# PaddlePaddle/PaddleNLP

Measured on AMD Instinct MI355X. Metric: tokens_per_sec_whole_node_llama3_8b_pretrain, higher is better.
Workload: dtype bf16; 1 GPU; model=llama3-8b, global_batch=8, seq_len=4096, parallelism=single, recompute=False

## Files before the change

### paddlenlp_amd/ops/csrc/bindings.cpp

```cpp
#include <torch/extension.h>
#include <ATen/hip/HIPContext.h>
#include <vector>

#include "launchers.h"

#define CHECK_GPU(x) TORCH_CHECK(x.is_cuda(), #x " must be on GPU")
#define CHECK_CONTIG(x) TORCH_CHECK(x.is_contiguous(), #x " must be contiguous")
#define CHECK_BF16(x) TORCH_CHECK(x.scalar_type() == torch::kBFloat16, #x " must be bf16")

static hipStream_t cur_stream() {
    return at::hip::getCurrentHIPStream().stream();
}

std::vector<torch::Tensor> rms_norm_fwd(torch::Tensor x, torch::Tensor w, double eps) {
    CHECK_GPU(x); CHECK_CONTIG(x); CHECK_BF16(x); CHECK_BF16(w);
    int H = x.size(-1);
    TORCH_CHECK(H % 8 == 0, "hidden size must be a multiple of 8");
    long long rows = x.numel() / H;
    auto y = torch::empty_like(x);
    auto invrms = torch::empty({rows}, x.options().dtype(torch::kFloat32));
    launch_rms_norm_fwd(x.data_ptr(), w.data_ptr(), y.data_ptr(),
                        invrms.data_ptr<float>(), rows, H, (float)eps, cur_stream());
    return {y, invrms};
}
// ... 141 lines not shown
        pre_lens.data_ptr<int>(), seq_lens.data_ptr<int>(),
        reinterpret_cast<const long long*>(eos_ids.data_ptr<int64_t>()),
        (int)eos_ids.numel(), not_need_stop.data_ptr<int>(),
        max_new ? max_new->data_ptr<int>() : nullptr,
        (long long)pad_id, B, (int)pre_ids.size(1), cur_stream());
}

void block_step(torch::Tensor block_table, torch::Tensor seq_lens,
                torch::Tensor stop_flags, torch::Tensor active,
                torch::Tensor free_list, torch::Tensor free_count,
                torch::Tensor is_block_step, int64_t block_size) {
    int B = block_table.size(0);
    launch_block_step(block_table.data_ptr<int>(), seq_lens.data_ptr<int>(),
                      stop_flags.data_ptr<signed char>(), active.data_ptr<signed char>(),
                      free_list.data_ptr<int>(), free_count.data_ptr<int>(),
                      is_block_step.data_ptr<signed char>(), B, (int)block_size,
                      (int)block_table.size(1), cur_stream());
}

torch::Tensor mfma32_probe(torch::Tensor A, torch::Tensor B) {
    CHECK_GPU(A); CHECK_BF16(A);
    auto C = torch::empty({32, 32}, A.options().dtype(torch::kFloat32));
    launch_mfma32_probe(A.contiguous().data_ptr(), B.contiguous().data_ptr(),
                        C.data_ptr<float>(), cur_stream());
    return C;
}

std::vector<torch::Tensor> permlane_probe() {
    auto opt = torch::TensorOptions().dtype(torch::kInt32).device(torch::kCUDA);
    auto o0 = torch::empty({64}, opt);
    auto o1 = torch::empty({64}, opt);
    launch_permlane_probe(o0.data_ptr<int>(), o1.data_ptr<int>(), cur_stream());
    return {o0, o1};
}

static void check_attn_args(const torch::Tensor& q, const torch::Tensor& k,
                            const torch::Tensor& v,
                            const torch::Tensor* dout = nullptr,
                            const torch::Tensor* o = nullptr,
                            const torch::Tensor* lse = nullptr,
                            const torch::Tensor* startend = nullptr) {
    auto check4d = [](const torch::Tensor& t, const char* name) {
        TORCH_CHECK(t.is_cuda(), name, " must be on GPU");
        TORCH_CHECK(t.scalar_type() == torch::kBFloat16, name, " must be bf16");
        TORCH_CHECK(t.is_contiguous(), name, " must be contiguous");
        TORCH_CHECK(t.dim() == 4, name, " must be [B,S,H,D]");
    };
    check4d(q, "q");
    check4d(k, "k");
    check4d(v, "v");
    int64_t B = q.size(0), Sq = q.size(1), Hq = q.size(2), D = q.size(3);
    int64_t Skv = k.size(1), Hk = k.size(2);
    TORCH_CHECK(D == 128 || D == 64 || D == 32, "head dim must be 32/64/128, got ", D);
    TORCH_CHECK(k.sizes() == v.sizes(), "k and v shapes must agree");
    TORCH_CHECK(k.size(0) == B && k.size(3) == D, "k/v must be [B,Skv,Hk,D] matching q");
    TORCH_CHECK(Hk > 0 && Hq % Hk == 0, "GQA requires Hq % Hk == 0");
    if (dout) {
        check4d(*dout, "dout");
        TORCH_CHECK(dout->sizes() == q.sizes(), "dout must be shaped like q");
    }
    if (o) {
        check4d(*o, "o");
        TORCH_CHECK(o->sizes() == q.sizes(), "o must be shaped like q");
    }
    if (lse) {
        TORCH_CHECK(lse->is_cuda() && lse->is_contiguous() &&
// ... 22 lines not shown
}

std::vector<torch::Tensor> flash_attn_fwd(torch::Tensor q, torch::Tensor k, torch::Tensor v,
                                          bool causal) {
    return flash_attn_fwd_ex(q, k, v, causal, false);
}

std::vector<torch::Tensor> flash_attn_bwd_ex(torch::Tensor dout, torch::Tensor q,
                                             torch::Tensor k, torch::Tensor v,
                                             torch::Tensor o, torch::Tensor lse,
                                             bool causal, bool force_v1) {
    check_attn_args(q, k, v, &dout, &o, &lse);
    int B = q.size(0), Sq = q.size(1), Hq = q.size(2), D = q.size(3);
    int Skv = k.size(1), Hk = k.size(2);
    auto dq = torch::empty_like(q);
    auto dk_h = torch::empty({B, Skv, Hk, D}, k.options());
    auto dv_h = torch::empty({B, Skv, Hk, D}, v.options());
    auto delta = torch::empty({B, Hq, Sq}, q.options().dtype(torch::kFloat32));
    float scale = 1.0f / std::sqrt((float)D);
    launch_flash_bwd(dout.data_ptr(), q.data_ptr(), k.data_ptr(), v.data_ptr(),
                     o.data_ptr(), lse.data_ptr<float>(), delta.data_ptr<float>(),
                     dq.data_ptr(), dk_h.data_ptr(), dv_h.data_ptr(),
                     B, Sq, Skv, Hq, Hk, D, scale, causal, force_v1, cur_stream());
    return {dq, dk_h, dv_h};
}

std::vector<torch::Tensor> flash_attn_bwd(torch::Tensor dout, torch::Tensor q,
                                          torch::Tensor k, torch::Tensor v,
                                          torch::Tensor o, torch::Tensor lse,
                                          bool causal) {
    return flash_attn_bwd_ex(dout, q, k, v, o, lse, causal, false);
}

void fused_adamw(std::vector<torch::Tensor> params, std::vector<torch::Tensor> grads,
                 std::vector<torch::Tensor> exp_avgs, std::vector<torch::Tensor> exp_avg_sqs,
                 std::vector<torch::Tensor> masters,
                 double lr, double beta1, double beta2, double eps, double wd,
                 int64_t step) {
    TORCH_CHECK(!params.empty());
    bool has_master = !masters.empty();
    const long long CHUNK = 1 << 22;
    std::vector<AdamWChunk> chunks;
    for (size_t i = 0; i < params.size(); i++) {
        auto& p = params[i];
        CHECK_GPU(p); CHECK_CONTIG(p);
        bool is_bf16 = p.scalar_type() == torch::kBFloat16;
        TORCH_CHECK(!is_bf16 || has_master, "bf16 params need master weights");
        long long n = p.numel();
        torch::Tensor g = grads[i];
        if (g.scalar_type() != p.scalar_type()) g = g.to(p.scalar_type());
        for (long long off = 0; off < n; off += CHUNK) {
            AdamWChunk c;
            c.param = p.data_ptr();
            c.grad = g.data_ptr();
            c.m = exp_avgs[i].data_ptr<float>();
            c.v = exp_avg_sqs[i].data_ptr<float>();
            c.master = has_master ? masters[i].data_ptr<float>() : nullptr;
            c.offset = off;
            c.n = std::min(CHUNK, n - off);
            c.is_bf16 = is_bf16 ? 1 : 0;
            chunks.push_back(c);
        }
    }
    auto meta = torch::from_blob(chunks.data(), {(long long)(chunks.size() * sizeof(AdamWChunk))},
                                 torch::kUInt8).clone();
    auto dev_meta = meta.to(params[0].device(), true);
// ... 136 lines not shown
    TORCH_CHECK(K % 8 == 0, "K must be a multiple of 8");
    auto y = torch::empty({R, (long)K}, x.options().dtype(torch::kFloat8_e4m3fn));
    auto scales = torch::empty({R}, x.options().dtype(torch::kFloat32));
    launch_fp8_rowwise_quant(x2.data_ptr(), y.data_ptr(), scales.data_ptr<float>(),
                             R, K, cur_stream());
    return {y, scales};
}

torch::Tensor wint8_gemv(torch::Tensor x, torch::Tensor wq, torch::Tensor scale) {
    CHECK_GPU(x); CHECK_BF16(x);
    auto x2 = x.contiguous().view({-1, x.size(-1)});
    int M = x2.size(0), K = x2.size(1), N = wq.size(0);
    TORCH_CHECK(M <= 16, "wint8_gemv is for decode shapes (M <= 16)");
    TORCH_CHECK(K % 128 == 0, "K must be a multiple of 128");
    auto sizes = x.sizes().vec();
    sizes.back() = N;
    auto y = torch::empty(sizes, x.options());
    launch_wint8_gemv(x2.data_ptr(), wq.data_ptr(), scale.data_ptr<float>(),
                      y.data_ptr(), M, N, K, cur_stream());
    return y;
}

PYBIND11_MODULE(TORCH_EXTENSION_NAME, m) {
    m.def("rms_norm_fwd", &rms_norm_fwd);
    m.def("rms_norm_bwd", &rms_norm_bwd);
    m.def("rope_fwd", &rope_fwd);
    m.def("swiglu_fwd", &swiglu_fwd);
    m.def("swiglu_bwd", &swiglu_bwd);
    m.def("cross_entropy_fwd", &cross_entropy_fwd);
    m.def("cross_entropy_bwd", &cross_entropy_bwd);
    m.def("mfma_probe", &mfma_probe);
    m.def("mfma32_probe", &mfma32_probe);
    m.def("permlane_probe", &permlane_probe);
    m.def("apply_repetition_penalty", &apply_repetition_penalty);
    m.def("topp_sample", &topp_sample,
          py::arg("logits"), py::arg("temperature"), py::arg("top_p"),
          py::arg("uniform"), py::arg("ban_eos") = py::none(),
          py::arg("cur_lens") = py::none(), py::arg("min_lens") = py::none());
    m.def("decode_update", &decode_update,
          py::arg("tokens"), py::arg("stop_flags"), py::arg("active"),
          py::arg("pre_ids"), py::arg("pre_lens"), py::arg("seq_lens"),
          py::arg("eos_ids"), py::arg("not_need_stop"),
          py::arg("max_new") = py::none(), py::arg("pad_id") = 0);
    m.def("block_step", &block_step);
    m.def("flash_attn_fwd", &flash_attn_fwd);
    m.def("flash_attn_fwd_ex", &flash_attn_fwd_ex);
    m.def("flash_attn_bwd", &flash_attn_bwd);
    m.def("flash_attn_bwd_ex", &flash_attn_bwd_ex);
    m.def("flashmask_attn_fwd", &flashmask_attn_fwd);
    m.def("flashmask_attn_bwd", &flashmask_attn_bwd);
    m.def("fused_adamw", &fused_adamw);
    m.def("paged_decode_attn", &paged_decode_attn,
          py::arg("q"), py::arg("k_cache"), py::arg("v_cache"),
          py::arg("block_table"), py::arg("seq_lens"),
          py::arg("k_scale") = c10::nullopt, py::arg("v_scale") = c10::nullopt);
    m.def("rope_cache_append", &rope_cache_append,
          py::arg("qkv"), py::arg("k_cache"), py::arg("v_cache"),
          py::arg("block_table"), py::arg("seq_lens_before"),
          py::arg("cos_t"), py::arg("sin_t"), py::arg("Hq"), py::arg("Hk"),
          py::arg("token_counts") = c10::nullopt,
          py::arg("k_scale") = c10::nullopt, py::arg("v_scale") = c10::nullopt);
    m.def("wint8_gemv", &wint8_gemv);
    m.def("fp8_rowwise_quant", &fp8_rowwise_quant);
    m.def("skinny_gemm", &skinny_gemm, py::arg("x"), py::arg("w"),
          py::arg("ksplit") = 8);
}
// ... 1 lines not shown
```

### paddlenlp_amd/ops/csrc/flash_attn_bwd_v2.hip

```cpp
#include "launchers.h"
#include "mfma.h"

#define FB2_WAVES 8
#define FB2_BLOCK (FB2_WAVES * 64)

template <int D, bool MASKED = false>
__global__ __launch_bounds__(FB2_BLOCK) void flash_bwd2_dq_kernel(
    const ushort_t* __restrict__ q, const ushort_t* __restrict__ k,
    const ushort_t* __restrict__ v, const ushort_t* __restrict__ dout,
    const float* __restrict__ lse, const float* __restrict__ delta,
    ushort_t* __restrict__ dq, const int* __restrict__ startend,
    int B, int Sq, int Skv, int Hq, int Hk, float scale, int causal) {
    constexpr int BLKN = 64;
    constexpr int DSTEPS = D / 16;
    constexpr int NDT = D / 32;
    constexpr int BLKM = FB2_WAVES * 32;

    __shared__ ushort_t k_lds[2][BLKN * D];
    __shared__ ushort_t v_lds[2][BLKN * D];
    __shared__ ushort_t kt_lds[2][D * BLKN];
    __shared__ int se_lds[2][MASKED ? BLKN : 1];

    const int tid = threadIdx.x;
    const int wave = tid >> 6;
    const int lane = tid & 63;
    const int l32 = lane & 31;
    const int hi = lane >> 5;

    int qt, bh;
    if ((gridDim.y & 7) == 0) {
        const int flat = blockIdx.x + gridDim.x * blockIdx.y;
        const int idx = flat >> 3;
        qt = idx % gridDim.x;
        bh = (flat & 7) * (gridDim.y >> 3) + idx / gridDim.x;
    } else {
        qt = blockIdx.x;
        bh = blockIdx.y;
    }
    const int b = bh / Hq, hq = bh % Hq;
    const int hk = hq / (Hq / Hk);
    const int q_base = qt * BLKM;
    const int qw = q_base + wave * 32;
    const int qg = qw + l32;
    const int causal_off = Skv - Sq;

    const long long q_row_stride = (long long)Hq * D;
    const long long kv_row_stride = (long long)Hk * D;
    const ushort_t* q_ptr = q + ((long long)b * Sq * Hq + hq) * D;
    const ushort_t* do_ptr = dout + ((long long)b * Sq * Hq + hq) * D;
    const ushort_t* k_ptr = k + ((long long)b * Skv * Hk + hk) * D;
    const ushort_t* v_ptr = v + ((long long)b * Skv * Hk + hk) * D;

    frag8 aq[DSTEPS], ado[DSTEPS];
    float lse_q = INFINITY, dl_q = 0.f;
    if (qg < Sq) {
#pragma unroll
        for (int kk = 0; kk < DSTEPS; kk++) {
            aq[kk] = *reinterpret_cast<const frag8*>(
                q_ptr + (long long)qg * q_row_stride + kk * 16 + hi * 8);
            ado[kk] = *reinterpret_cast<const frag8*>(
                do_ptr + (long long)qg * q_row_stride + kk * 16 + hi * 8);
        }
        lse_q = lse[((long long)b * Hq + hq) * Sq + qg];
        dl_q = delta[((long long)b * Hq + hq) * Sq + qg];
    } else {
#pragma unroll
        for (int kk = 0; kk < DSTEPS; kk++) { aq[kk] = frag8{0}; ado[kk] = frag8{0}; }
    }

    f32x16 acc_dq[NDT];
#pragma unroll
// ... 113 lines not shown
            if (MASKED) {
                se_max_next = tile_se_max(kv_base + BLKN);
                stage_skip = (q_base >= se_max_next);
            }
            if (!stage_skip) load_tile(kv_base + BLKN);
        }
        if (!wave_skip) process_sub(1);

        if (kvt + 1 < n_kv_tiles && !stage_skip)
            write_tile(cur ^ 1, kv_base + BLKN);
        if (MASKED) se_max_cur = se_max_next;
        __syncthreads();
    }

#pragma unroll
    for (int r = 0; r < 16; r++) {
        int qrow = qw + crow32(r, hi);
        if (qrow >= Sq) continue;
        ushort_t* dqr = dq + ((long long)b * Sq + qrow) * q_row_stride + (long long)hq * D;
#pragma unroll
        for (int n = 0; n < NDT; n++)
            dqr[n * 32 + l32] = f32_to_bf16(acc_dq[n][r]);
    }
}

template <int D, bool MASKED = false>
__global__ __launch_bounds__(FB2_BLOCK, 1) void flash_bwd2_dkv_kernel(
    const ushort_t* __restrict__ q, const ushort_t* __restrict__ k,
    const ushort_t* __restrict__ v, const ushort_t* __restrict__ dout,
    const float* __restrict__ lse, const float* __restrict__ delta,
    ushort_t* __restrict__ dk, ushort_t* __restrict__ dv,
    const int* __restrict__ startend,
    int B, int Sq, int Skv, int Hq, int Hk, float scale, int causal) {
    constexpr int BLKQ = 64;
    constexpr int DSTEPS = D / 16;
    constexpr int NDT = D / 32;
    constexpr int BLKKV = FB2_WAVES * 32;

    __shared__ ushort_t q_lds[2][BLKQ * D];
    __shared__ ushort_t do_lds[2][BLKQ * D];
    __shared__ ushort_t qt_lds[2][D * BLKQ];
    __shared__ ushort_t dot_lds[2][D * BLKQ];
    __shared__ float lse_lds[2][BLKQ];
    __shared__ float dl_lds[2][BLKQ];

    const int tid = threadIdx.x;
    const int wave = tid >> 6;
    const int lane = tid & 63;
    const int l32 = lane & 31;
    const int hi = lane >> 5;

    int kvt, bh;
    if ((gridDim.y & 7) == 0) {
        const int flat = blockIdx.x + gridDim.x * blockIdx.y;
        const int idx = flat >> 3;
        kvt = idx % gridDim.x;
        bh = (flat & 7) * (gridDim.y >> 3) + idx / gridDim.x;
    } else {
        kvt = blockIdx.x;
        bh = blockIdx.y;
    }
    const int b = bh / Hk, hk = bh % Hk;
    const int G = Hq / Hk;
    const int kv_base = kvt * BLKKV;
    const int kvw = kv_base + wave * 32;
    const int kvg_lane = kvw + l32;
    const int causal_off = Skv - Sq;
    __shared__ int blk_max_lds[MASKED ? FB2_WAVES : 1];
    int kv_end_lane = 0x7fffffff;
    int wave_max_end = 0x7fffffff;
    int block_max_end = 0x7fffffff;
    if (MASKED) {
        kv_end_lane = (kvg_lane < Skv)
            ? startend[(long long)b * Skv + kvg_lane] : 0;
        wave_max_end = kv_end_lane;
#pragma unroll
        for (int off = 32; off; off >>= 1)
            wave_max_end = max(wave_max_end,
                               __shfl_xor(wave_max_end, off, 64));
        if (lane == 0) blk_max_lds[wave] = wave_max_end;
    }

    const long long q_row_stride = (long long)Hq * D;
    const long long kv_row_stride = (long long)Hk * D;
    const ushort_t* k_ptr = k + ((long long)b * Skv * Hk + hk) * D;
    const ushort_t* v_ptr = v + ((long long)b * Skv * Hk + hk) * D;

    frag8 bk[DSTEPS], bv[DSTEPS];
    if (kvg_lane < Skv) {
#pragma unroll
        for (int kk = 0; kk < DSTEPS; kk++) {
            bk[kk] = *reinterpret_cast<const frag8*>(
                k_ptr + (long long)kvg_lane * kv_row_stride + kk * 16 + hi * 8);
            bv[kk] = *reinterpret_cast<const frag8*>(
                v_ptr + (long long)kvg_lane * kv_row_stride + kk * 16 + hi * 8);
        }
    } else {
#pragma unroll
        for (int kk = 0; kk < DSTEPS; kk++) { bk[kk] = frag8{0}; bv[kk] = frag8{0}; }
    }

    f32x16 acc_dk[NDT], acc_dv[NDT];
#pragma unroll
    for (int n = 0; n < NDT; n++)
#pragma unroll
        for (int r = 0; r < 16; r++) { acc_dk[n][r] = 0.f; acc_dv[n][r] = 0.f; }

    int qt0 = 0;
    if (causal) qt0 = max(0, (kv_base - causal_off) / BLKQ);
    const int n_q_tiles = (Sq + BLKQ - 1) / BLKQ;

    const int s_rowp = tid >> 4;
    const int s_col = (tid & 15) * 8;
    const int s_row0 = s_rowp * 2;
    short8v sq0, sq1, sd0, sd1;

    for (int g = 0; g < G; g++) {
        const int hq = hk * G + g;
        const ushort_t* q_ptr = q + ((long long)b * Sq * Hq + hq) * D;
        const ushort_t* do_ptr = dout + ((long long)b * Sq * Hq + hq) * D;
        const float* lse_row = lse + ((long long)b * Hq + hq) * Sq;
        const float* dl_row = delta + ((long long)b * Hq + hq) * Sq;

        auto load_qtile = [&](int q_tb) {
            int g0 = q_tb + s_row0;
            sq0 = short8v{0,0,0,0,0,0,0,0}; sq1 = sq0; sd0 = sq0; sd1 = sq0;
            if (g0 < Sq) {
                sq0 = *reinterpret_cast<const short8v*>(q_ptr + (long long)g0 * q_row_stride + s_col);
                sd0 = *reinterpret_cast<const short8v*>(do_ptr + (long long)g0 * q_row_stride + s_col);
            }
            if (g0 + 1 < Sq) {
                sq1 = *reinterpret_cast<const short8v*>(q_ptr + (long long)(g0 + 1) * q_row_stride + s_col);
                sd1 = *reinterpret_cast<const short8v*>(do_ptr + (long long)(g0 + 1) * q_row_stride + s_col);
            }
        };
        auto write_qtile = [&](int q_tb, int buf) {
            *reinterpret_cast<short8v*>(swz<D>(q_lds[buf], s_row0, s_col)) = sq0;
            *reinterpret_cast<short8v*>(swz<D>(q_lds[buf], s_row0 + 1, s_col)) = sq1;
            *reinterpret_cast<short8v*>(swz<D>(do_lds[buf], s_row0, s_col)) = sd0;
            *reinterpret_cast<short8v*>(swz<D>(do_lds[buf], s_row0 + 1, s_col)) = sd1;
#pragma unroll
            for (int j = 0; j < 8; j++) {
                unsigned pq = ((unsigned)(unsigned short)sq0[j]) |
                              (((unsigned)(unsigned short)sq1[j]) << 16);
                unsigned pd = ((unsigned)(unsigned short)sd0[j]) |
                              (((unsigned)(unsigned short)sd1[j]) << 16);
                *reinterpret_cast<unsigned*>(swz<BLKQ>(qt_lds[buf], s_col + j, s_row0)) = pq;
                *reinterpret_cast<unsigned*>(swz<BLKQ>(dot_lds[buf], s_col + j, s_row0)) = pd;
            }
            if (tid < BLKQ) {
                int qgl = q_tb + tid;
                lse_lds[buf][tid] = (qgl < Sq) ? lse_row[qgl] : INFINITY;
                dl_lds[buf][tid] = (qgl < Sq) ? dl_row[qgl] : 0.f;
            }
        };

        load_qtile(qt0 * BLKQ);
        write_qtile(qt0 * BLKQ, qt0 & 1);
        __syncthreads();
        if (MASKED) {
            block_max_end = blk_max_lds[0];
#pragma unroll
            for (int w = 1; w < FB2_WAVES; w++)
                block_max_end = max(block_max_end, blk_max_lds[w]);
        }

        for (int qt = qt0; qt < n_q_tiles; qt++) {
            const int q_tb = qt * BLKQ;
            const int cur = qt & 1;
            bool wave_skip =
                causal && (q_tb + BLKQ - 1 + causal_off < kvw);
            if (MASKED && q_tb >= wave_max_end) wave_skip = true;

            if (!wave_skip) {
#pragma unroll 1
                for (int sub = 0; sub < 2; sub++) {
                    f32x16 st, dp;
#pragma unroll
                    for (int r = 0; r < 16; r++) { st[r] = 0.f; dp[r] = 0.f; }
                    __builtin_amdgcn_s_setprio(1);
#pragma unroll
                    for (int kk = 0; kk < DSTEPS; kk++) {
                        frag8 aqf = *reinterpret_cast<const frag8*>(
                            swz<D>(q_lds[cur], sub * 32 + l32, kk * 16 + hi * 8));
                        frag8 adf = *reinterpret_cast<const frag8*>(
                            swz<D>(do_lds[cur], sub * 32 + l32, kk * 16 + hi * 8));
                        st = mfma32(aqf, bk[kk], st);
                        dp = mfma32(adf, bv[kk], dp);
                    }
                    __builtin_amdgcn_s_setprio(0);

#pragma unroll
                    for (int r = 0; r < 16; r++) {
                        int qrow = sub * 32 + crow32(r, hi);
                        int qgl = q_tb + qrow;
                        float ls = lse_lds[cur][qrow];
                        float dl = dl_lds[cur][qrow];
                        bool vis = (qgl < Sq) && (kvg_lane < Skv) &&
                                   (!causal || kvg_lane <= qgl + causal_off);
                        if (MASKED) vis = vis && (qgl < kv_end_lane);
                        float p = (vis && ls != INFINITY)
                                      ? __expf(st[r] * scale - ls) : 0.f;
                        st[r] = p;
                        dp[r] = p * (dp[r] - dl) * scale;
                    }

                    __builtin_amdgcn_s_setprio(1);
#pragma unroll
                    for (int ksl = 0; ksl < 2; ksl++) {
                        const int ks = sub * 2 + ksl;
                        frag8 apt = t12_convert(st, ksl * 8);
                        frag8 ads = t12_convert(dp, ksl * 8);
#pragma unroll
                        for (int n = 0; n < NDT; n++) {
                            frag8 bdo = *reinterpret_cast<const frag8*>(
                                swz<BLKQ>(dot_lds[cur], n * 32 + l32, ks * 16 + hi * 8));
                            frag8 bq = *reinterpret_cast<const frag8*>(
                                swz<BLKQ>(qt_lds[cur], n * 32 + l32, ks * 16 + hi * 8));
                            acc_dv[n] = mfma32(apt, bdo, acc_dv[n]);
                            acc_dk[n] = mfma32(ads, bq, acc_dk[n]);
                        }
                    }
                    __builtin_amdgcn_s_setprio(0);
                }
            }

            if (qt + 1 < n_q_tiles &&
                !(MASKED && q_tb + BLKQ >= block_max_end)) {
                load_qtile(q_tb + BLKQ);
                write_qtile(q_tb + BLKQ, cur ^ 1);
            }
            __syncthreads();
        }
        __syncthreads();
    }

    const long long out_row_stride = (long long)Hk * D;
#pragma unroll
    for (int r = 0; r < 16; r++) {
        int kvr = kvw + crow32(r, hi);
        if (kvr >= Skv) continue;
        long long base = ((long long)b * Skv + kvr) * out_row_stride + (long long)hk * D;
#pragma unroll
        for (int n = 0; n < NDT; n++) {
            dk[base + n * 32 + l32] = f32_to_bf16(acc_dk[n][r]);
            dv[base + n * 32 + l32] = f32_to_bf16(acc_dv[n][r]);
        }
    }
}

bool launch_flash_bwd2(const void* dout, const void* q, const void* k, const void* v,
                       const void* o, const float* lse, float* delta,
                       void* dq, void* dk, void* dv,
                       int B, int Sq, int Skv, int Hq, int Hk, int D,
                       float scale, bool causal, hipStream_t stream) {
    if (D != 128 || (Hq % Hk) != 0) return false;
    launch_flash_bwd_delta(dout, o, delta, B, Sq, Hq, D, stream);
    dim3 gq((Sq + 255) / 256, B * Hq);
    hipLaunchKernelGGL((flash_bwd2_dq_kernel<128, false>), gq, dim3(FB2_BLOCK), 0, stream,
                       (const ushort_t*)q, (const ushort_t*)k, (const ushort_t*)v,
                       (const ushort_t*)dout, lse, delta, (ushort_t*)dq,
                       (const int*)nullptr,
                       B, Sq, Skv, Hq, Hk, scale, causal ? 1 : 0);
    dim3 gkv((Skv + 255) / 256, B * Hk);
    hipLaunchKernelGGL((flash_bwd2_dkv_kernel<128, false>), gkv, dim3(FB2_BLOCK), 0, stream,
                       (const ushort_t*)q, (const ushort_t*)k, (const ushort_t*)v,
                       (const ushort_t*)dout, lse, delta, (ushort_t*)dk, (ushort_t*)dv,
                       (const int*)nullptr,
                       B, Sq, Skv, Hq, Hk, scale, causal ? 1 : 0);
    return true;
}

bool launch_flash_bwd2_mask(const void* dout, const void* q, const void* k,
                            const void* v, const void* o, const float* lse,
                            float* delta, void* dq, void* dk, void* dv,
                            const int* startend,
                            int B, int Sq, int Skv, int Hq, int Hk, int D,
                            float scale, hipStream_t stream) {
    if (D != 128 || (Hq % Hk) != 0) return false;
    launch_flash_bwd_delta(dout, o, delta, B, Sq, Hq, D, stream);
    dim3 gq((Sq + 255) / 256, B * Hq);
    hipLaunchKernelGGL((flash_bwd2_dq_kernel<128, true>), gq, dim3(FB2_BLOCK), 0, stream,
                       (const ushort_t*)q, (const ushort_t*)k, (const ushort_t*)v,
                       (const ushort_t*)dout, lse, delta, (ushort_t*)dq, startend,
                       B, Sq, Skv, Hq, Hk, scale, 1);
    dim3 gkv((Skv + 255) / 256, B * Hk);
    hipLaunchKernelGGL((flash_bwd2_dkv_kernel<128, true>), gkv, dim3(FB2_BLOCK), 0, stream,
                       (const ushort_t*)q, (const ushort_t*)k, (const ushort_t*)v,
                       (const ushort_t*)dout, lse, delta, (ushort_t*)dk, (ushort_t*)dv,
                       startend, B, Sq, Skv, Hq, Hk, scale, 1);
    return true;
}
```

### paddlenlp_amd/ops/csrc/flash_attn_v2.hip

```cpp
#include "launchers.h"
#include "mfma.h"

#define FA2_WAVES 8
#define FA2_BLOCK (FA2_WAVES * 64)
#define FA2_BLKN 64
#define FA2_QW 32
#define FA2_BLKM (FA2_WAVES * FA2_QW)
#define DEFER_THR 8.0f

__global__ void mfma32_layout_probe(const ushort_t* A, const ushort_t* B, float* C) {
    int l = threadIdx.x;
    int l32 = l & 31, hi = l >> 5;
    frag8 a, b;
#pragma unroll
    for (int j = 0; j < 8; j++) {
        a[j] = (short)A[l32 * 16 + hi * 8 + j];
        b[j] = (short)B[(hi * 8 + j) * 32 + l32];
    }
    f32x16 c;
#pragma unroll
    for (int r = 0; r < 16; r++) c[r] = 0.f;
    c = mfma32(a, b, c);
#pragma unroll
    for (int r = 0; r < 16; r++) C[crow32(r, hi) * 32 + l32] = c[r];
// ... 1 lines not shown

__global__ void permlane_probe(int* out0, int* out1) {
    int l = threadIdx.x;
    auto r = __builtin_amdgcn_permlane32_swap((unsigned)l, (unsigned)(1000 + l),
                                              false, false);
    out0[l] = (int)r[0];
    out1[l] = (int)r[1];
}

template <int D, bool MASKED = false>
__global__ __launch_bounds__(FA2_BLOCK) void flash_fwd2_kernel(
    const ushort_t* __restrict__ q,
    const ushort_t* __restrict__ k,
    const ushort_t* __restrict__ v,
    ushort_t* __restrict__ o,
    float* __restrict__ lse,
    const int* __restrict__ startend,
    int B, int Sq, int Skv, int Hq, int Hk, float scale, int causal) {
    constexpr int DSTEPS = D / 16;
    constexpr int NDT = D / 32;
    constexpr int KVT = FA2_BLKN / 32;

    __shared__ ushort_t k_lds[2][FA2_BLKN * D];
    __shared__ ushort_t vt_lds[2][D * FA2_BLKN];
    __shared__ int se_lds[2][MASKED ? FA2_BLKN : 1];

    const int tid = threadIdx.x;
    const int wave = tid >> 6;
    const int lane = tid & 63;
    const int l32 = lane & 31;
    const int hi = lane >> 5;

    int qt, bh;
    if ((gridDim.y & 7) == 0) {
        const int flat = blockIdx.x + gridDim.x * blockIdx.y;
        const int idx = flat >> 3;
        qt = idx % gridDim.x;
        bh = (flat & 7) * (gridDim.y >> 3) + idx / gridDim.x;
    } else {
        qt = blockIdx.x;
        bh = blockIdx.y;
    }
    const int b = bh / Hq, hq = bh % Hq;
    const int hk = hq / (Hq / Hk);
    const int q_base = qt * FA2_BLKM;
    const int qw = q_base + wave * FA2_QW;
    const int qg = qw + l32;
    const int causal_off = Skv - Sq;

    const long long q_row_stride = (long long)Hq * D;
    const long long kv_row_stride = (long long)Hk * D;
    const ushort_t* q_ptr = q + ((long long)b * Sq * Hq + hq) * D;
    const ushort_t* k_ptr = k + ((long long)b * Skv * Hk + hk) * D;
    const ushort_t* v_ptr = v + ((long long)b * Skv * Hk + hk) * D;

    frag8 aq[DSTEPS];
    if (qg < Sq) {
#pragma unroll
        for (int kk = 0; kk < DSTEPS; kk++)
            aq[kk] = *reinterpret_cast<const frag8*>(
                q_ptr + (long long)qg * q_row_stride + kk * 16 + hi * 8);
    } else {
#pragma unroll
        for (int kk = 0; kk < DSTEPS; kk++) aq[kk] = frag8{0};
    }

    float m_run = -INFINITY, l_run = 0.f;
    f32x16 acc_o[NDT];
#pragma unroll
    for (int n = 0; n < NDT; n++)
#pragma unroll
        for (int r = 0; r < 16; r++) acc_o[n][r] = 0.f;

    int n_kv_tiles = (Skv + FA2_BLKN - 1) / FA2_BLKN;
    if (causal) {
// ... 236 lines not shown
```

### paddlenlp_amd/ops/csrc/launchers.h

```cpp
#pragma once

#include <hip/hip_runtime_api.h>

#include <stdexcept>
#include <string>

[[noreturn]] inline void unsupported_head_dim(const char* op, int D) {
    throw std::runtime_error(std::string(op) + ": no kernel for head dim " +
                             std::to_string(D));
}

void launch_rms_norm_fwd(const void* x, const void* w, void* y, float* invrms,
                         long long rows, int H, float eps, hipStream_t stream);
void launch_rms_norm_bwd(const void* dy, const void* x, const void* w,
                         const float* invrms, void* dx, float* dw_partial,
                         float* dw32, void* dw, bool dw_is_bf16,
                         long long rows, int H, int P, hipStream_t stream);
void launch_rope(const void* x, void* out, const float* cos_t, const float* sin_t,
                 long long n_rows, int H, int D, int S, bool backward,
                 hipStream_t stream);
void launch_swiglu_fwd(const void* x, void* y, long long N, int I, hipStream_t stream);
void launch_swiglu_bwd(const void* dy, const void* x, void* dx, long long N, int I,
                       hipStream_t stream);
void launch_ce_fwd(const void* logits, const long long* labels, float* loss,
// ... 10 lines not shown
    float* v;
    float* master;
    long long offset;
    long long n;
    int is_bf16;
};
void launch_adamw(const AdamWChunk* dev_chunks, int n_chunks,
                  float lr, float beta1, float beta2, float eps, float wd,
                  float bias1, float bias2, hipStream_t stream);

void launch_mfma_probe(const void* A, const void* B, float* C, hipStream_t stream);
void launch_flash_fwd(const void* q, const void* k, const void* v, void* o,
                      float* lse, int B, int Sq, int Skv, int Hq, int Hk, int D,
                      float scale, bool causal, bool force_v1, hipStream_t stream);
void launch_flash_bwd(const void* dout, const void* q, const void* k, const void* v,
                      const void* o, const float* lse, float* delta,
                      void* dq, void* dk, void* dv,
                      int B, int Sq, int Skv, int Hq, int Hk, int D,
                      float scale, bool causal, bool force_v1, hipStream_t stream);
void launch_flash_fwd_mask(const void* q, const void* k, const void* v, void* o,
                           float* lse, const int* startend,
                           int B, int Sq, int Skv, int Hq, int Hk, int D,
                           float scale, hipStream_t stream);
void launch_flash_bwd_mask(const void* dout, const void* q, const void* k, const void* v,
                           const void* o, const float* lse, float* delta,
                           void* dq, void* dk, void* dv, const int* startend,
                           int B, int Sq, int Skv, int Hq, int Hk, int D,
                           float scale, hipStream_t stream);
void launch_flash_bwd_delta(const void* dout, const void* o, float* delta,
                            int B, int Sq, int Hq, int D, hipStream_t stream);

void launch_mfma32_probe(const void* A, const void* B, float* C, hipStream_t stream);
void launch_permlane_probe(int* out0, int* out1, hipStream_t stream);
bool launch_flash_fwd2(const void* q, const void* k, const void* v, void* o,
                       float* lse, int B, int Sq, int Skv, int Hq, int Hk,
                       int D, float scale, bool causal, hipStream_t stream);
bool launch_flash_fwd2_mask(const void* q, const void* k, const void* v,
                            void* o, float* lse, const int* startend,
                            int B, int Sq, int Skv, int Hq, int Hk,
                            int D, float scale, hipStream_t stream);
bool launch_flash_bwd2(const void* dout, const void* q, const void* k, const void* v,
                       const void* o, const float* lse, float* delta,
                       void* dq, void* dk, void* dv,
                       int B, int Sq, int Skv, int Hq, int Hk, int D,
                       float scale, bool causal, hipStream_t stream);
bool launch_flash_bwd2_mask(const void* dout, const void* q, const void* k,
                            const void* v, const void* o, const float* lse,
                            float* delta, void* dq, void* dk, void* dv,
                            const int* startend,
                            int B, int Sq, int Skv, int Hq, int Hk, int D,
                            float scale, hipStream_t stream);

int paged_decode_nsplit(int B, int Hk);
void launch_paged_decode_attn(const void* q, const void* k_cache, const void* v_cache,
                              const float* k_scale, const float* v_scale,
                              const int* block_table, const int* seq_lens, void* out,
                              float* partials, int nsplit,
                              int B, int Hq, int Hk, int D, int block_size,
                              int max_blocks, float scale, int cache_mode,
                              hipStream_t stream);
bool launch_paged_decode_attn3(const void* q, const void* k_cache, const void* v_cache,
                               const float* k_scale, const float* v_scale,
                               const int* block_table, const int* seq_lens, void* out,
                               float* partials, int nsplit,
                               int B, int Hq, int Hk, int D, int block_size,
                               int max_blocks, float scale, int cache_mode,
                               hipStream_t stream);
void launch_rope_cache_append(const void* qkv, void* q_out, void* k_cache, void* v_cache,
                              float* k_scale, float* v_scale,
                              const int* block_table, const int* seq_lens_before,
                              const float* cos_t, const float* sin_t,
                              int B, int T, int Hq, int Hk, int D, int block_size,
                              int max_blocks, const int* token_counts,
                              int cache_mode, hipStream_t stream);

void launch_wint8_gemv(const void* x, const void* wq, const float* scale, void* y,
                       int M, int N, int K, hipStream_t stream);
void launch_fp8_rowwise_quant(const void* x, void* y, float* scales,
// ... 24 lines not shown
```

### paddlenlp_amd/ops/csrc/mfma.h

```cpp
#pragma once

#include "common.h"

typedef short8v frag8;

__device__ __forceinline__ f32x4 mfma16(frag8 a, frag8 b, f32x4 c) {
    return __builtin_amdgcn_mfma_f32_16x16x32_bf16(a, b, c, 0, 0, 0);
}

__device__ __forceinline__ f32x16 mfma32(frag8 a, frag8 b, f32x16 c) {
    return __builtin_amdgcn_mfma_f32_32x32x16_bf16(a, b, c, 0, 0, 0);
}

__device__ __forceinline__ int crow32(int r, int hi) {
    return (r & 3) + 8 * (r >> 2) + 4 * hi;
}

template <int LD>
__device__ __forceinline__ char* swz(ushort_t* base, int row, int col_elem) {
    return reinterpret_cast<char*>(base) +
           (((row * LD + col_elem) * 2) ^ ((row & 7) << 4));
}

__device__ __forceinline__ unsigned pack_bf16(float a, float b) {
    return (unsigned)f32_to_bf16(a) | ((unsigned)f32_to_bf16(b) << 16);
}

__device__ __forceinline__ frag8 t12_convert(const f32x16& p, int rb) {
    unsigned w[4];
    {
        unsigned lo0 = pack_bf16(p[rb + 0], p[rb + 1]);
        unsigned hi0 = pack_bf16(p[rb + 4], p[rb + 5]);
        auto rr = __builtin_amdgcn_permlane32_swap(lo0, hi0, false, false);
        w[0] = rr[0]; w[2] = rr[1];
    }
    {
        unsigned lo1 = pack_bf16(p[rb + 2], p[rb + 3]);
        unsigned hi1 = pack_bf16(p[rb + 6], p[rb + 7]);
        auto rr = __builtin_amdgcn_permlane32_swap(lo1, hi1, false, false);
        w[1] = rr[0]; w[3] = rr[1];
    }
    frag8 f;
#pragma unroll
    for (int j = 0; j < 4; j++) {
        f[j * 2] = (short)(w[j] & 0xffff);
        f[j * 2 + 1] = (short)(w[j] >> 16);
    }
    return f;
}
```

Measured before the change: 19380 tokens/s.

## Use LDS DMA and transpose reads in flash bwd dKV; regroup XCD tile order

The dK/dV backward kernel now fills one swizzled shared-memory image per Q and dO tile using direct global-to-LDS DMA loads. It reads transposed fragments with ds_read_tr16 instead of storing separate row and transposed copies through registers. The loop over heads and Q tiles is flattened into one double-buffered pipeline that prefetches the next tile, and the masked case computes the upper bound on Q tiles once. Block-to-tile mapping across XCDs is regrouped so head groups are interleaved, with descending tile order for forward and dQ and ascending for dKV. A probe kernel and a parts-selectable backward entry point are also added.

Measured after the change: 21080 tokens/s (median of 6 runs). +8.7%, better.

```diff
diff --git a/paddlenlp_amd/ops/csrc/bindings.cpp b/paddlenlp_amd/ops/csrc/bindings.cpp
--- a/paddlenlp_amd/ops/csrc/bindings.cpp
+++ b/paddlenlp_amd/ops/csrc/bindings.cpp
@@ -197,6 +197,18 @@
     auto o1 = torch::empty({64}, opt);
     launch_permlane_probe(o0.data_ptr<int>(), o1.data_ptr<int>(), cur_stream());
     return {o0, o1};
+}
+
+std::vector<torch::Tensor> lds_image_probe(torch::Tensor X) {
+    CHECK_GPU(X); CHECK_BF16(X);
+    TORCH_CHECK(X.dim() == 2 && X.size(0) == 64 && X.size(1) == 128,
+                "lds_image_probe: X must be [64,128]");
+    auto Xc = X.contiguous();
+    auto out_row = torch::empty_like(Xc);
+    auto out_tr = torch::empty_like(Xc);
+    launch_lds_image_probe(Xc.data_ptr(), out_row.data_ptr(), out_tr.data_ptr(),
+                           cur_stream());
+    return {out_row, out_tr};
 }
 
 static void check_attn_args(const torch::Tensor& q, const torch::Tensor& k,
@@ -285,6 +297,31 @@
     return flash_attn_bwd_ex(dout, q, k, v, o, lse, causal, false);
 }
 
+std::vector<torch::Tensor> flash_attn_bwd2_parts(torch::Tensor dout, torch::Tensor q,
+                                                 torch::Tensor k, torch::Tensor v,
+                                                 torch::Tensor o, torch::Tensor lse,
+                                                 torch::Tensor delta, bool causal,
+                                                 int64_t parts) {
+    check_attn_args(q, k, v, &dout, &o, &lse);
+    TORCH_CHECK(delta.is_cuda() && delta.is_contiguous() &&
+                    delta.scalar_type() == torch::kFloat32 &&
+                    delta.sizes() == lse.sizes(),
+                "delta must be a contiguous fp32 GPU tensor shaped like lse");
+    int B = q.size(0), Sq = q.size(1), Hq = q.size(2), D = q.size(3);
+    int Skv = k.size(1), Hk = k.size(2);
+    auto dq = torch::empty_like(q);
+    auto dk_h = torch::empty({B, Skv, Hk, D}, k.options());
+    auto dv_h = torch::empty({B, Skv, Hk, D}, v.options());
+    float scale = 1.0f / std::sqrt((float)D);
+    TORCH_CHECK(launch_flash_bwd2(dout.data_ptr(), q.data_ptr(), k.data_ptr(),
+                                  v.data_ptr(), o.data_ptr(), lse.data_ptr<float>(),
+                                  delta.data_ptr<float>(), dq.data_ptr(),
+                                  dk_h.data_ptr(), dv_h.data_ptr(), B, Sq, Skv, Hq,
+                                  Hk, D, scale, causal, cur_stream(), (int)parts),
+                "flash_attn_bwd2_parts: no v2 kernel for this shape");
+    return {dq, dk_h, dv_h};
+}
+
 void fused_adamw(std::vector<torch::Tensor> params, std::vector<torch::Tensor> grads,
                  std::vector<torch::Tensor> exp_avgs, std::vector<torch::Tensor> exp_avg_sqs,
                  std::vector<torch::Tensor> masters,
@@ -487,6 +524,8 @@
     m.def("mfma_probe", &mfma_probe);
     m.def("mfma32_probe", &mfma32_probe);
     m.def("permlane_probe", &permlane_probe);
+    m.def("lds_image_probe", &lds_image_probe);
+    m.def("flash_attn_bwd2_parts", &flash_attn_bwd2_parts);
     m.def("apply_repetition_penalty", &apply_repetition_penalty);
     m.def("topp_sample", &topp_sample,
           py::arg("logits"), py::arg("temperature"), py::arg("top_p"),
diff --git a/paddlenlp_amd/ops/csrc/flash_attn_bwd_v2.hip b/paddlenlp_amd/ops/csrc/flash_attn_bwd_v2.hip
--- a/paddlenlp_amd/ops/csrc/flash_attn_bwd_v2.hip
+++ b/paddlenlp_amd/ops/csrc/flash_attn_bwd_v2.hip
@@ -28,15 +28,7 @@
     const int hi = lane >> 5;
 
     int qt, bh;
-    if ((gridDim.y & 7) == 0) {
-        const int flat = blockIdx.x + gridDim.x * blockIdx.y;
-        const int idx = flat >> 3;
-        qt = idx % gridDim.x;
-        bh = (flat & 7) * (gridDim.y >> 3) + idx / gridDim.x;
-    } else {
-        qt = blockIdx.x;
-        bh = blockIdx.y;
-    }
+    xcd_grouped_tile<FA_ORDER_W, false>(qt, bh);
     const int b = bh / Hq, hq = bh % Hq;
     const int hk = hq / (Hq / Hk);
     const int q_base = qt * BLKM;
@@ -216,34 +208,23 @@
     ushort_t* __restrict__ dk, ushort_t* __restrict__ dv,
     const int* __restrict__ startend,
     int B, int Sq, int Skv, int Hq, int Hk, float scale, int causal) {
+    static_assert(D == 128, "the dual-use image is laid out for 128-column tiles");
     constexpr int BLKQ = 64;
     constexpr int DSTEPS = D / 16;
     constexpr int NDT = D / 32;
     constexpr int BLKKV = FB2_WAVES * 32;
 
-    __shared__ ushort_t q_lds[2][BLKQ * D];
-    __shared__ ushort_t do_lds[2][BLKQ * D];
-    __shared__ ushort_t qt_lds[2][D * BLKQ];
-    __shared__ ushort_t dot_lds[2][D * BLKQ];
-    __shared__ float lse_lds[2][BLKQ];
-    __shared__ float dl_lds[2][BLKQ];
+    __shared__ __attribute__((aligned(16))) ushort_t qd_lds[2][2][BLKQ * D];
+    __shared__ float ld_lds[2][2][BLKQ];
 
     const int tid = threadIdx.x;
-    const int wave = tid >> 6;
+    const int wave = __builtin_amdgcn_readfirstlane(tid >> 6);
     const int lane = tid & 63;
     const int l32 = lane & 31;
     const int hi = lane >> 5;
 
     int kvt, bh;
-    if ((gridDim.y & 7) == 0) {
-        const int flat = blockIdx.x + gridDim.x * blockIdx.y;
-        const int idx = flat >> 3;
-        kvt = idx % gridDim.x;
-        bh = (flat & 7) * (gridDim.y >> 3) + idx / gridDim.x;
-    } else {
-        kvt = blockIdx.x;
-        bh = blockIdx.y;
-    }
+    xcd_grouped_tile<FA_ORDER_W, true>(kvt, bh);
     const int b = bh / Hk, hk = bh % Hk;
     const int G = Hq / Hk;
     const int kv_base = kvt * BLKKV;
@@ -253,7 +234,6 @@
     __shared__ int blk_max_lds[MASKED ? FB2_WAVES : 1];
     int kv_end_lane = 0x7fffffff;
     int wave_max_end = 0x7fffffff;
-    int block_max_end = 0x7fffffff;
     if (MASKED) {
         kv_end_lane = (kvg_lane < Skv)
             ? startend[(long long)b * Skv + kvg_lane] : 0;
@@ -262,6 +242,7 @@
         for (int off = 32; off; off >>= 1)
             wave_max_end = max(wave_max_end,
                                __shfl_xor(wave_max_end, off, 64));
+        wave_max_end = __builtin_amdgcn_readfirstlane(wave_max_end);
         if (lane == 0) blk_max_lds[wave] = wave_max_end;
     }
 
@@ -292,131 +273,113 @@
 
     int qt0 = 0;
     if (causal) qt0 = max(0, (kv_base - causal_off) / BLKQ);
-    const int n_q_tiles = (Sq + BLKQ - 1) / BLKQ;
-
-    const int s_rowp = tid >> 4;
-    const int s_col = (tid & 15) * 8;
-    const int s_row0 = s_rowp * 2;
-    short8v sq0, sq1, sd0, sd1;
-
-    for (int g = 0; g < G; g++) {
+    int qt_end = (Sq + BLKQ - 1) / BLKQ;
+    if (MASKED) {
+        __syncthreads();
+        int block_max_end = blk_max_lds[0];
+#pragma unroll
+        for (int w = 1; w < FB2_WAVES; w++)
+            block_max_end = max(block_max_end, blk_max_lds[w]);
+        block_max_end = __builtin_amdgcn_readfirstlane(block_max_end);
+        if (block_max_end < Sq)
+            qt_end = (max(block_max_end, 0) + BLKQ - 1) / BLKQ;
+    }
+    const int n_tiles = G * max(qt_end - qt0, 0);
+
+    auto issue_tile = [&](int g, int qt, int buf) {
         const int hq = hk * G + g;
-        const ushort_t* q_ptr = q + ((long long)b * Sq * Hq + hq) * D;
-        const ushort_t* do_ptr = dout + ((long long)b * Sq * Hq + hq) * D;
-        const float* lse_row = lse + ((long long)b * Hq + hq) * Sq;
-        const float* dl_row = delta + ((long long)b * Hq + hq) * Sq;
-
-        auto load_qtile = [&](int q_tb) {
-            int g0 = q_tb + s_row0;
-            sq0 = short8v{0,0,0,0,0,0,0,0}; sq1 = sq0; sd0 = sq0; sd1 = sq0;
-            if (g0 < Sq) {
-                sq0 = *reinterpret_cast<const short8v*>(q_ptr + (long long)g0 * q_row_stride + s_col);
-                sd0 = *reinterpret_cast<const short8v*>(do_ptr + (long long)g0 * q_row_stride + s_col);
+        const long long head_off = ((long long)b * Sq * Hq + hq) * D;
+        const int q_tb = qt * BLKQ;
+        const int ln = fresh_lane_id();
+#pragma unroll
+        for (int i = 0; i < 2; i++) {
+            const int piece = wave * 2 + i;
+            const int src_row = min(q_tb + img_fill_row(piece, ln), Sq - 1);
+            const long long src = head_off + (long long)src_row * q_row_stride +
+                                  img_fill_chunk(piece, ln) * 8;
+            lds_dma16(q + src, &qd_lds[buf][0][piece * 512]);
+            lds_dma16(dout + src, &qd_lds[buf][1][piece * 512]);
+        }
+        if (wave < 2) {
+            const float* row = (wave == 0 ? lse : delta) +
+                               ((long long)b * Hq + hq) * Sq;
+            lds_dma4(row + min(q_tb + ln, Sq - 1), &ld_lds[buf][wave][0]);
+        }
+    };
+
+    int g_next = 0, qt_next = qt0;
+    auto advance_next = [&]() {
+        if (++qt_next == qt_end) { qt_next = qt0; g_next++; }
+    };
+#pragma unroll
+    for (int kk = 0; kk < DSTEPS; kk++)
+        asm volatile("" :: "v"(bk[kk]), "v"(bv[kk]));
+    if (n_tiles > 0) { issue_tile(g_next, qt_next, 0); advance_next(); }
+
+    int qt = qt0;
+    for (int t = 0; t < n_tiles; t++) {
+        const int cur = t & 1;
+        lds_dma_wait_all();
+        __syncthreads();
+        if (t + 1 < n_tiles) { issue_tile(g_next, qt_next, cur ^ 1); advance_next(); }
+
+        const int q_tb = qt * BLKQ;
+        const ushort_t* q_img = qd_lds[cur][0];
+        const ushort_t* do_img = qd_lds[cur][1];
+        const int lane_t = fresh_lane_id();
+        bool wave_skip =
+            causal && (q_tb + BLKQ - 1 + causal_off < kvw);
+        if (MASKED && q_tb >= wave_max_end) wave_skip = true;
+
+        if (!wave_skip) {
+#pragma unroll 1
+            for (int sub = 0; sub < 2; sub++) {
+                f32x16 st, dp;
+#pragma unroll
+                for (int r = 0; r < 16; r++) { st[r] = 0.f; dp[r] = 0.f; }
+                __builtin_amdgcn_s_setprio(1);
+#pragma unroll
+                for (int kk = 0; kk < DSTEPS; kk++) {
+                    frag8 aqf = img_row_frag(q_img, sub * 32 + l32, kk, hi);
+                    frag8 adf = img_row_frag(do_img, sub * 32 + l32, kk, hi);
+                    st = mfma32(aqf, bk[kk], st);
+                    dp = mfma32(adf, bv[kk], dp);
+                }
+                __builtin_amdgcn_s_setprio(0);
+
+#pragma unroll
+                for (int r = 0; r < 16; r++) {
+                    int qrow = sub * 32 + crow32(r, hi);
+                    int qgl = q_tb + qrow;
+                    float ls = ld_lds[cur][0][qrow];
+                    float dl = ld_lds[cur][1][qrow];
+                    bool vis = (qgl < Sq) && (kvg_lane < Skv) &&
+                               (!causal || kvg_lane <= qgl + causal_off);
+                    if (MASKED) vis = vis && (qgl < kv_end_lane);
+                    float p = (vis && ls != INFINITY)
+                                  ? __expf(st[r] * scale - ls) : 0.f;
+                    st[r] = p;
+                    dp[r] = p * (dp[r] - dl) * scale;
+                }
+
+                __builtin_amdgcn_s_setprio(1);
+#pragma unroll
+                for (int ksl = 0; ksl < 2; ksl++) {
+                    const int ks = sub * 2 + ksl;
+                    frag8 apt = t12_convert(st, ksl * 8);
+                    frag8 ads = t12_convert(dp, ksl * 8);
+#pragma unroll
+                    for (int n = 0; n < NDT; n++) {
+                        frag8 bdo = img_tr_frag(do_img, ks, n, lane_t);
+                        frag8 bq = img_tr_frag(q_img, ks, n, lane_t);
+                        acc_dv[n] = mfma32(apt, bdo, acc_dv[n]);
+                        acc_dk[n] = mfma32(ads, bq, acc_dk[n]);
+                    }
+                }
+                __builtin_amdgcn_s_setprio(0);
             }
-            if (g0 + 1 < Sq) {
-                sq1 = *reinterpret_cast<const short8v*>(q_ptr + (long long)(g0 + 1) * q_row_stride + s_col);
-                sd1 = *reinterpret_cast<const short8v*>(do_ptr + (long long)(g0 + 1) * q_row_stride + s_col);
-            }
-        };
-        auto write_qtile = [&](int q_tb, int buf) {
-            *reinterpret_cast<short8v*>(swz<D>(q_lds[buf], s_row0, s_col)) = sq0;
-            *reinterpret_cast<short8v*>(swz<D>(q_lds[buf], s_row0 + 1, s_col)) = sq1;
-            *reinterpret_cast<short8v*>(swz<D>(do_lds[buf], s_row0, s_col)) = sd0;
-            *reinterpret_cast<short8v*>(swz<D>(do_lds[buf], s_row0 + 1, s_col)) = sd1;
-#pragma unroll
-            for (int j = 0; j < 8; j++) {
-                unsigned pq = ((unsigned)(unsigned short)sq0[j]) |
-                              (((unsigned)(unsigned short)sq1[j]) << 16);
-                unsigned pd = ((unsigned)(unsigned short)sd0[j]) |
-                              (((unsigned)(unsigned short)sd1[j]) << 16);
-                *reinterpret_cast<unsigned*>(swz<BLKQ>(qt_lds[buf], s_col + j, s_row0)) = pq;
-                *reinterpret_cast<unsigned*>(swz<BLKQ>(dot_lds[buf], s_col + j, s_row0)) = pd;
-            }
-            if (tid < BLKQ) {
-                int qgl = q_tb + tid;
-                lse_lds[buf][tid] = (qgl < Sq) ? lse_row[qgl] : INFINITY;
-                dl_lds[buf][tid] = (qgl < Sq) ? dl_row[qgl] : 0.f;
-            }
-        };
-
-        load_qtile(qt0 * BLKQ);
-        write_qtile(qt0 * BLKQ, qt0 & 1);
-        __syncthreads();
-        if (MASKED) {
-            block_max_end = blk_max_lds[0];
-#pragma unroll
-            for (int w = 1; w < FB2_WAVES; w++)
-                block_max_end = max(block_max_end, blk_max_lds[w]);
-        }
-
-        for (int qt = qt0; qt < n_q_tiles; qt++) {
-            const int q_tb = qt * BLKQ;
-            const int cur = qt & 1;
-            bool wave_skip =
-                causal && (q_tb + BLKQ - 1 + causal_off < kvw);
-            if (MASKED && q_tb >= wave_max_end) wave_skip = true;
-
-            if (!wave_skip) {
-#pragma unroll 1
-                for (int sub = 0; sub < 2; sub++) {
-                    f32x16 st, dp;
-#pragma unroll
-                    for (int r = 0; r < 16; r++) { st[r] = 0.f; dp[r] = 0.f; }
-                    __builtin_amdgcn_s_setprio(1);
-#pragma unroll
-                    for (int kk = 0; kk < DSTEPS; kk++) {
-                        frag8 aqf = *reinterpret_cast<const frag8*>(
-                            swz<D>(q_lds[cur], sub * 32 + l32, kk * 16 + hi * 8));
-                        frag8 adf = *reinterpret_cast<const frag8*>(
-                            swz<D>(do_lds[cur], sub * 32 + l32, kk * 16 + hi * 8));
-                        st = mfma32(aqf, bk[kk], st);
-                        dp = mfma32(adf, bv[kk], dp);
-                    }
-                    __builtin_amdgcn_s_setprio(0);
-
-#pragma unroll
-                    for (int r = 0; r < 16; r++) {
-                        int qrow = sub * 32 + crow32(r, hi);
-                        int qgl = q_tb + qrow;
-                        float ls = lse_lds[cur][qrow];
-                        float dl = dl_lds[cur][qrow];
-                        bool vis = (qgl < Sq) && (kvg_lane < Skv) &&
-                                   (!causal || kvg_lane <= qgl + causal_off);
-                        if (MASKED) vis = vis && (qgl < kv_end_lane);
-                        float p = (vis && ls != INFINITY)
-                                      ? __expf(st[r] * scale - ls) : 0.f;
-                        st[r] = p;
-                        dp[r] = p * (dp[r] - dl) * scale;
-                    }
-
-                    __builtin_amdgcn_s_setprio(1);
-#pragma unroll
-                    for (int ksl = 0; ksl < 2; ksl++) {
-                        const int ks = sub * 2 + ksl;
-                        frag8 apt = t12_convert(st, ksl * 8);
-                        frag8 ads = t12_convert(dp, ksl * 8);
-#pragma unroll
-                        for (int n = 0; n < NDT; n++) {
-                            frag8 bdo = *reinterpret_cast<const frag8*>(
-                                swz<BLKQ>(dot_lds[cur], n * 32 + l32, ks * 16 + hi * 8));
-                            frag8 bq = *reinterpret_cast<const frag8*>(
-                                swz<BLKQ>(qt_lds[cur], n * 32 + l32, ks * 16 + hi * 8));
-                            acc_dv[n] = mfma32(apt, bdo, acc_dv[n]);
-                            acc_dk[n] = mfma32(ads, bq, acc_dk[n]);
-                        }
-                    }
-                    __builtin_amdgcn_s_setprio(0);
-                }
-            }
-
-            if (qt + 1 < n_q_tiles &&
-                !(MASKED && q_tb + BLKQ >= block_max_end)) {
-                load_qtile(q_tb + BLKQ);
-                write_qtile(q_tb + BLKQ, cur ^ 1);
-            }
-            __syncthreads();
-        }
-        __syncthreads();
+        }
+        if (++qt == qt_end) qt = qt0;
     }
 
     const long long out_row_stride = (long long)Hk * D;
@@ -433,25 +396,63 @@
     }
 }
 
+__global__ __launch_bounds__(64) void lds_image_probe(
+    const ushort_t* __restrict__ X, ushort_t* __restrict__ out_row,
+    ushort_t* __restrict__ out_tr) {
+    __shared__ __attribute__((aligned(16))) ushort_t img[64 * 128];
+    const int lane = threadIdx.x;
+    const int l32 = lane & 31, hi = lane >> 5;
+#pragma unroll 1
+    for (int piece = 0; piece < 16; piece++)
+        lds_dma16(X + img_fill_row(piece, lane) * 128 + img_fill_chunk(piece, lane) * 8,
+                  &img[piece * 512]);
+    lds_dma_wait_all();
+    __syncthreads();
+    for (int sub = 0; sub < 2; sub++)
+        for (int kk = 0; kk < 8; kk++) {
+            frag8 f = img_row_frag(img, sub * 32 + l32, kk, hi);
+            *reinterpret_cast<frag8*>(
+                out_row + (sub * 32 + l32) * 128 + kk * 16 + hi * 8) = f;
+        }
+    for (int ks = 0; ks < 4; ks++)
+        for (int n = 0; n < 4; n++) {
+            frag8 f = img_tr_frag(img, ks, n, lane);
+#pragma unroll
+            for (int j = 0; j < 8; j++)
+                out_tr[(ks * 16 + hi * 8 + j) * 128 + n * 32 + l32] = (ushort_t)f[j];
+        }
+}
+
+void launch_lds_image_probe(const void* X, void* out_row, void* out_tr,
+                            hipStream_t stream) {
+    hipLaunchKernelGGL(lds_image_probe, dim3(1), dim3(64), 0, stream,
+                       (const ushort_t*)X, (ushort_t*)out_row, (ushort_t*)out_tr);
+}
+
 bool launch_flash_bwd2(const void* dout, const void* q, const void* k, const void* v,
                        const void* o, const float* lse, float* delta,
                        void* dq, void* dk, void* dv,
                        int B, int Sq, int Skv, int Hq, int Hk, int D,
-                       float scale, bool causal, hipStream_t stream) {
+                       float scale, bool causal, hipStream_t stream, int parts) {
     if (D != 128 || (Hq % Hk) != 0) return false;
-    launch_flash_bwd_delta(dout, o, delta, B, Sq, Hq, D, stream);
-    dim3 gq((Sq + 255) / 256, B * Hq);
-    hipLaunchKernelGGL((flash_bwd2_dq_kernel<128, false>), gq, dim3(FB2_BLOCK), 0, stream,
-                       (const ushort_t*)q, (const ushort_t*)k, (const ushort_t*)v,
-                       (const ushort_t*)dout, lse, delta, (ushort_t*)dq,
-                       (const int*)nullptr,
-                       B, Sq, Skv, Hq, Hk, scale, causal ? 1 : 0);
-    dim3 gkv((Skv + 255) / 256, B * Hk);
-    hipLaunchKernelGGL((flash_bwd2_dkv_kernel<128, false>), gkv, dim3(FB2_BLOCK), 0, stream,
-                       (const ushort_t*)q, (const ushort_t*)k, (const ushort_t*)v,
-                       (const ushort_t*)dout, lse, delta, (ushort_t*)dk, (ushort_t*)dv,
-                       (const int*)nullptr,
-                       B, Sq, Skv, Hq, Hk, scale, causal ? 1 : 0);
+    if (parts & FLASH_BWD_DELTA)
+        launch_flash_bwd_delta(dout, o, delta, B, Sq, Hq, D, stream);
+    if (parts & FLASH_BWD_DQ) {
+        dim3 gq((Sq + 255) / 256, B * Hq);
+        hipLaunchKernelGGL((flash_bwd2_dq_kernel<128, false>), gq, dim3(FB2_BLOCK), 0, stream,
+                           (const ushort_t*)q, (const ushort_t*)k, (const ushort_t*)v,
+                           (const ushort_t*)dout, lse, delta, (ushort_t*)dq,
+                           (const int*)nullptr,
+                           B, Sq, Skv, Hq, Hk, scale, causal ? 1 : 0);
+    }
+    if (parts & FLASH_BWD_DKV) {
+        dim3 gkv((Skv + 255) / 256, B * Hk);
+        hipLaunchKernelGGL((flash_bwd2_dkv_kernel<128, false>), gkv, dim3(FB2_BLOCK), 0, stream,
+                           (const ushort_t*)q, (const ushort_t*)k, (const ushort_t*)v,
+                           (const ushort_t*)dout, lse, delta, (ushort_t*)dk, (ushort_t*)dv,
+                           (const int*)nullptr,
+                           B, Sq, Skv, Hq, Hk, scale, causal ? 1 : 0);
+    }
     return true;
 }
 
diff --git a/paddlenlp_amd/ops/csrc/flash_attn_v2.hip b/paddlenlp_amd/ops/csrc/flash_attn_v2.hip
--- a/paddlenlp_amd/ops/csrc/flash_attn_v2.hip
+++ b/paddlenlp_amd/ops/csrc/flash_attn_v2.hip
@@ -57,15 +57,7 @@
     const int hi = lane >> 5;
 
     int qt, bh;
-    if ((gridDim.y & 7) == 0) {
-        const int flat = blockIdx.x + gridDim.x * blockIdx.y;
-        const int idx = flat >> 3;
-        qt = idx % gridDim.x;
-        bh = (flat & 7) * (gridDim.y >> 3) + idx / gridDim.x;
-    } else {
-        qt = blockIdx.x;
-        bh = blockIdx.y;
-    }
+    xcd_grouped_tile<FA_ORDER_W, false>(qt, bh);
     const int b = bh / Hq, hq = bh % Hq;
     const int hk = hq / (Hq / Hk);
     const int q_base = qt * FA2_BLKM;
diff --git a/paddlenlp_amd/ops/csrc/launchers.h b/paddlenlp_amd/ops/csrc/launchers.h
--- a/paddlenlp_amd/ops/csrc/launchers.h
+++ b/paddlenlp_amd/ops/csrc/launchers.h
@@ -66,6 +66,8 @@
 
 void launch_mfma32_probe(const void* A, const void* B, float* C, hipStream_t stream);
 void launch_permlane_probe(int* out0, int* out1, hipStream_t stream);
+void launch_lds_image_probe(const void* X, void* out_row, void* out_tr,
+                            hipStream_t stream);
 bool launch_flash_fwd2(const void* q, const void* k, const void* v, void* o,
                        float* lse, int B, int Sq, int Skv, int Hq, int Hk,
                        int D, float scale, bool causal, hipStream_t stream);
@@ -73,11 +75,13 @@
                             void* o, float* lse, const int* startend,
                             int B, int Sq, int Skv, int Hq, int Hk,
                             int D, float scale, hipStream_t stream);
+enum { FLASH_BWD_DELTA = 1, FLASH_BWD_DQ = 2, FLASH_BWD_DKV = 4, FLASH_BWD_ALL = 7 };
 bool launch_flash_bwd2(const void* dout, const void* q, const void* k, const void* v,
                        const void* o, const float* lse, float* delta,
                        void* dq, void* dk, void* dv,
                        int B, int Sq, int Skv, int Hq, int Hk, int D,
-                       float scale, bool causal, hipStream_t stream);
+                       float scale, bool causal, hipStream_t stream,
+                       int parts = FLASH_BWD_ALL);
 bool launch_flash_bwd2_mask(const void* dout, const void* q, const void* k,
                             const void* v, const void* o, const float* lse,
                             float* delta, void* dq, void* dk, void* dv,
diff --git a/paddlenlp_amd/ops/csrc/mfma.h b/paddlenlp_amd/ops/csrc/mfma.h
--- a/paddlenlp_amd/ops/csrc/mfma.h
+++ b/paddlenlp_amd/ops/csrc/mfma.h
@@ -48,3 +48,86 @@
     }
     return f;
 }
+
+__device__ __forceinline__ int img_off(int row, int ch) {
+    return 2048 * (row >> 3) + 512 * (ch >> 2) + 64 * (row & 7) +
+           16 * ((ch & 3) ^ ((row >> 2) & 3));
+}
+
+typedef short short4v __attribute__((ext_vector_type(4)));
+typedef __attribute__((address_space(3))) short4v lds_short4v;
+
+__device__ __forceinline__ int img_fill_row(int piece, int lane) {
+    return 8 * (piece >> 1) + ((lane >> 2) & 7);
+}
+__device__ __forceinline__ int img_fill_chunk(int piece, int lane) {
+    const int row = img_fill_row(piece, lane);
+    return 4 * (2 * (piece & 1) + (lane >> 5)) + ((lane & 3) ^ ((row >> 2) & 3));
+}
+__device__ __forceinline__ unsigned lds_addr(const void* p) {
+    return (unsigned)(unsigned long long)p;
+}
+__device__ __forceinline__ void lds_dma16(const void* src, const void* lds_dst) {
+    unsigned keep;
+    asm volatile("s_mov_b32 %0, m0\n\ts_mov_b32 m0, %2\n\ts_nop 0\n\t"
+                 "global_load_lds_dwordx4 %1, off\n\ts_mov_b32 m0, %0"
+                 : "=&s"(keep) : "v"(src), "s"(lds_addr(lds_dst)) : "memory");
+}
+__device__ __forceinline__ void lds_dma4(const void* src, const void* lds_dst) {
+    unsigned keep;
+    asm volatile("s_mov_b32 %0, m0\n\ts_mov_b32 m0, %2\n\ts_nop 0\n\t"
+                 "global_load_lds_dword %1, off\n\ts_mov_b32 m0, %0"
+                 : "=&s"(keep) : "v"(src), "s"(lds_addr(lds_dst)) : "memory");
+}
+__device__ __forceinline__ void lds_dma_wait_all() {
+    asm volatile("s_waitcnt vmcnt(0)" ::: "memory");
+}
+
+__device__ __forceinline__ frag8 img_row_frag(const ushort_t* img, int row, int kk, int hi) {
+    return *reinterpret_cast<const frag8*>(
+        reinterpret_cast<const char*>(img) + img_off(row, kk * 2 + hi));
+}
+
+__device__ __forceinline__ frag8 img_tr_frag(const ushort_t* img, int ks, int n, int lane) {
+    const int i = lane & 15, qq = i >> 2, p = i & 3;
+    const int hi = lane >> 5;
+    const int c0 = n * 4 + ((lane >> 4) & 1) * 2 + (p >> 1);
+    const char* base = reinterpret_cast<const char*>(img) + 8 * (p & 1);
+    frag8 f;
+#pragma unroll
+    for (int jj = 0; jj < 2; jj++) {
+        const int row = ks * 16 + hi * 8 + jj * 4 + qq;
+        short4v t = __builtin_amdgcn_ds_read_tr16_b64_v4i16(
+            (lds_short4v*)(base + img_off(row, c0)));
+#pragma unroll
+        for (int e = 0; e < 4; e++) f[jj * 4 + e] = t[e];
+    }
+    return f;
+}
+
+__device__ __forceinline__ int fresh_lane_id() {
+    int ln;
+    asm volatile("v_mbcnt_lo_u32_b32 %0, -1, 0\n\tv_mbcnt_hi_u32_b32 %0, -1, %0"
+                 : "=v"(ln));
+    return ln;
+}
+
+#define FA_ORDER_W 4
+template <int W, bool ASCENDING>
+__device__ __forceinline__ void xcd_grouped_tile(int& tile, int& bh) {
+    const int T = gridDim.x;
+    if ((gridDim.y & 7) != 0) {
+        tile = blockIdx.x;
+        bh = blockIdx.y;
+        return;
+    }
+    const int flat = blockIdx.x + T * blockIdx.y;
+    const int idx = flat >> 3;
+    const int hp = gridDim.y >> 3;
+    const int grp = idx / (W * T);
+    const int rem = idx - grp * (W * T);
+    const int wg = min(W, hp - grp * W);
+    const int rank = rem / wg;
+    tile = ASCENDING ? rank : T - 1 - rank;
+    bh = (flat & 7) * hp + grp * W + (rem - rank * wg);
+}
```
